# codebydant/sfM_danPipeline

Measured on AMD Instinct MI355X. Metric: image-pairs matched/sec + BA iterations/sec (200 cams, 100k pts, 1M obs), higher is better.
Workload: dtype i8

## Files before the change

### sfm_danpipeline_amd/csrc/match.hip

```cpp
#include "common.h"
#include <type_traits>
#include <vector>
#include <algorithm>
#include <string.h>
#include <stdlib.h>

namespace {

typedef int v4i __attribute__((ext_vector_type(4)));
typedef int v16i __attribute__((ext_vector_type(16)));

enum { KIND_F32_L2 = 0, KIND_U8_L2 = 1, KIND_U8_HAMMING = 2 };

constexpr int TILE_ROWS = 32;
constexpr int HPAD = -(1 << 23);
constexpr int TAG_BITS = 8;
constexpr int EPOCH_TILES = 1 << TAG_BITS;
constexpr int TAG_MASK = EPOCH_TILES - 1;
constexpr int FIX_FLAG = 1 << 30;
constexpr int FIX_GRID = 1024;
constexpr int FIX_CAP = 1 << 20;
constexpr int DIST_EMPTY = 0x7FFFFFFF;
constexpr int KNN_WAVES = 4;
constexpr int HCHUNK = 1024;
// ... 24 lines not shown
  int* par;
  int* nodd;
  int n_rows;
  int n_pad;
};

struct WorkItem {
  int pair;
  int qtile0;
  int qimg, timg;
};

template <int NC>
__host__ __device__ constexpr int chunk_pos(int r, int c) {
  constexpr int SH = (NC == 16) ? 0 : (NC == 8) ? 1 : (NC == 4) ? 2 : 3;
  return r * NC + (c ^ ((r >> SH) & (NC - 1)));
}
__device__ __forceinline__ int imax3(int a, int b, int c) { return max(max(a, b), c); }
__device__ __forceinline__ int imed3(int a, int b, int c) { return max(min(a, b), min(max(a, b), c)); }

template <int KIND>
__global__ __launch_bounds__(256) void parity_kernel(const ImgDev* __restrict__ imgs, const int* __restrict__ tile_img,
                                                     const int* __restrict__ tile_first, int dim) {
  const int img = tile_img[blockIdx.x];
  const int tile = blockIdx.x - tile_first[img];
  const ImgDev I = imgs[img];
  const int l = threadIdx.x & 31;
#pragma unroll
  for (int rr = 0; rr < 4; ++rr) {
    const int row = tile * TILE_ROWS + rr * 8 + (threadIdx.x >> 5);
    int s = 0;
    if (row < I.n_rows) {
      if (KIND == KIND_F32_L2) {
        const float* src = (const float*)I.raw + (size_t)row * dim;
        for (int k = l; k < dim; k += 32) {
          const float f = src[k];
          int x = (int)f;
          x = x < 0 ? 0 : (x > 255 ? 255 : x);
          s ^= x;
        }
      } else {
        const unsigned char* src = (const unsigned char*)I.raw + (size_t)row * dim;
        for (int k = l; k < dim; k += 32) s ^= src[k];
      }
    }
#pragma unroll
    for (int o = 1; o < 32; o <<= 1) s ^= __shfl_xor(s, o);
    if (l == 0 && row < I.n_pad) I.par[row] = (row < I.n_rows) ? (s & 1) : 0;
  }
}

__global__ __launch_bounds__(256) void order_kernel(const ImgDev* __restrict__ imgs, int by_parity) {
  __shared__ int wsum[4];
  __shared__ int run_odd, run_even, n_odd_pad_s;
  const ImgDev I = imgs[blockIdx.x];
  const int lane = threadIdx.x & 63, wave = threadIdx.x >> 6;
  for (int p = threadIdx.x; p < I.n_pad; p += 256) I.perm[p] = (!by_parity && p < I.n_rows) ? p : -1;
  if (!by_parity) {
    if (threadIdx.x == 0) *I.nodd = 0;
    return;
  }
  int c = 0;
  for (int r = threadIdx.x; r < I.n_rows; r += 256) c += I.par[r];
#pragma unroll
  for (int o = 1; o < 64; o <<= 1) c += __shfl_xor(c, o);
  if (lane == 0) wsum[wave] = c;
  __syncthreads();
  if (threadIdx.x == 0) {
    const int n_odd = wsum[0] + wsum[1] + wsum[2] + wsum[3];
    n_odd_pad_s = (n_odd + TILE_ROWS - 1) / TILE_ROWS * TILE_ROWS;
    *I.nodd = n_odd_pad_s;
    run_odd = 0;
    run_even = 0;
  }
  __syncthreads();
  const int n_odd_pad = n_odd_pad_s;
  for (int r0 = 0; r0 < I.n_rows; r0 += 256) {
    const int r = r0 + threadIdx.x;
    const bool valid = r < I.n_rows;
    const bool odd = valid && I.par[r];
    const unsigned long long bo = __ballot(odd), bv = __ballot(valid);
    const unsigned long long below = (1ull << lane) - 1ull;
    if (lane == 0) wsum[wave] = __popcll(bo) | (__popcll(bv) << 16);
    __syncthreads();
    int odd_before = run_odd, valid_before = 0;
    for (int w = 0; w < wave; ++w) {
      odd_before += wsum[w] & 0xFFFF;
      valid_before += wsum[w] >> 16;
    }
    const int my_odd = odd_before + __popcll(bo & below);
    const int my_valid = valid_before + __popcll(bv & below);
    if (valid) {
      const int even_before = run_even + (my_valid - (my_odd - run_odd));
      I.perm[odd ? my_odd : n_odd_pad + even_before] = r;
    }
    __syncthreads();
    if (threadIdx.x == 0) {
      int so = 0, sv = 0;
      for (int w = 0; w < 4; ++w) {
        so += wsum[w] & 0xFFFF;
        sv += wsum[w] >> 16;
      }
      run_odd += so;
      run_even += sv - so;
    }
    __syncthreads();
  }
}

template <int KS, int KIND>
__global__ void prepare_kernel(const ImgDev* __restrict__ imgs, const int* __restrict__ tile_img,
                               const int* __restrict__ tile_first, int dim, int* __restrict__ nonintegral,
                               int gen) {
  constexpr int NC = 2 * KS;
  constexpr int RB = 32 * KS;
  const int img = tile_img[blockIdx.x];
  const int tile = blockIdx.x - tile_first[img];
  const ImgDev I = imgs[img];
  const int r = threadIdx.x / NC, c = threadIdx.x % NC;
  const int pos = tile * TILE_ROWS + r;
  const int row = I.perm[pos];
  const bool valid = row >= 0;
  signed char v[16];
  int n2 = 0;
  bool ok = true;
  if (KIND == KIND_U8_HAMMING) {
    const int nbits = dim * 8;
    unsigned bits = 0;
    if (valid) {
      const unsigned char* src = (const unsigned char*)I.raw + (size_t)row * dim;
      const int b0 = 2 * c;
      if (b0 < dim) bits |= src[b0];
      if (b0 + 1 < dim) bits |= (unsigned)src[b0 + 1] << 8;
    }
#pragma unroll
    for (int e = 0; e < 16; ++e) {
      const int k = c * 16 + e;
      v[e] = (valid && k < nbits) ? (((bits >> e) & 1u) ? 8 : -8) : 0;
    }
  } else {
    float fv[16];
    unsigned char bv[16];
    const bool full = valid && c * 16 + 16 <= dim;
    if (KIND == KIND_F32_L2) {
      const float* src = (const float*)I.raw + (size_t)(valid ? row : 0) * dim + c * 16;
      if (full && (((size_t)src) & 15) == 0) {
        typedef float v4f __attribute__((ext_vector_type(4)));
// ... 15 lines not shown
      if (full && (((size_t)src) & 15) == 0) {
        const v4i x = *(g_v4i_p)src;
        memcpy(bv, &x, 16);
      } else {
#pragma unroll
        for (int e = 0; e < 16; ++e) bv[e] = (valid && c * 16 + e < dim) ? src[e] : 128;
      }
    }
#pragma unroll
    for (int e = 0; e < 16; ++e) {
      const int k = c * 16 + e;
      int x = 128;
      if (valid && k < dim) {
        if (KIND == KIND_F32_L2) {
          const float f = fv[e];
          ok = ok && (f == rintf(f)) && (f >= 0.f) && (f <= 255.f);
          x = (int)f;
          x = x < 0 ? 0 : (x > 255 ? 255 : x);
        } else {
          x = bv[e];
        }
      }
      const int cv = x - 128;
      v[e] = (signed char)cv;
      n2 += cv * cv;
    }
  }
#pragma unroll
  for (int o = 1; o < NC; o <<= 1) n2 += __shfl_xor(n2, o);
  int4 out;
  memcpy(&out, v, 16);
  int4* dst = (int4*)(I.tiles + (size_t)tile * (TILE_ROWS * RB)) + chunk_pos<NC>(r, c);
  *dst = out;
  if (c == 0) {
    int ci;
    if (KIND == KIND_U8_HAMMING)
      ci = ((valid ? dim * 8 * (HCHUNK / 2) : (dim * 8 + 1) * HCHUNK)) | (pos & (HCHUNK - 1));
    else ci = valid ? -((n2 + 1) >> 1) : HPAD;
    I.cin[pos] = ci;
    I.nq[pos] = valid ? n2 : 0;
  }
  if (KIND == KIND_F32_L2 && !ok) nonintegral[img] = gen;
}

template <int NC>
__device__ __forceinline__ int group_sum(int x) {
  if (NC >= 2) x += __builtin_amdgcn_update_dpp(0, x, 0xB1, 0xF, 0xF, true);
  if (NC >= 4) x += __builtin_amdgcn_update_dpp(0, x, 0x4E, 0xF, 0xF, true);
  if (NC >= 8) x += __builtin_amdgcn_update_dpp(0, x, 0x141, 0xF, 0xF, true);
  if (NC >= 16) x += __builtin_amdgcn_update_dpp(0, x, 0x140, 0xF, 0xF, true);
  return x;
}

struct Best2 {
  int d0, i0, x0, d1, i1, x1;
};
__device__ __forceinline__ bool lex_less(int da, int ia, int db, int ib) { return da < db || (da == db && ia < ib); }
__device__ __forceinline__ void best2_insert(Best2& b, int d, int i, int x) {
  if (lex_less(d, i, b.d0, b.i0)) {
    b.d1 = b.d0;
    b.i1 = b.i0;
    b.x1 = b.x0;
    b.d0 = d;
    b.i0 = i;
    b.x0 = x;
  } else if (lex_less(d, i, b.d1, b.i1)) {
    b.d1 = d;
    b.i1 = i;
    b.x1 = x;
  }
}

template <int I>
__device__ __forceinline__ void epi_op(const v16i& D0, const v16i& D1, int (&sl)[16], int& k0, int& k1, int (&T)[16],
                                       int tag0, int tag1) {
  if constexpr (I < 16) {
    sl[I] = imax3(sl[I], D0[I], D1[I]);
  } else {
    constexpr int J = (I - 16) % 11;
    constexpr int B = (I - 16) < 11 ? 0 : 8;
    const v16i& D = (I - 16) < 11 ? D0 : D1;
    const int tag = (I - 16) < 11 ? tag0 : tag1;
    if constexpr (J == 0) T[B + 0] = imax3(D[0], D[1], D[2]);
    if constexpr (J == 1) T[B + 1] = imax3(D[3], D[4], D[5]);
    if constexpr (J == 2) T[B + 2] = imax3(D[6], D[7], D[8]);
    if constexpr (J == 3) T[B + 3] = imax3(D[9], D[10], D[11]);
    if constexpr (J == 4) T[B + 4] = imax3(D[12], D[13], D[14]);
    if constexpr (J == 5) T[B + 5] = imax3(T[B + 0], T[B + 1], T[B + 2]);
    if constexpr (J == 6) T[B + 6] = imax3(T[B + 3], T[B + 4], D[15]);
    if constexpr (J == 7) T[B + 7] = max(T[B + 5], T[B + 6]);
    if constexpr (J == 8) T[B + 7] = (T[B + 7] << TAG_BITS) | tag;
    if constexpr (J == 9) k1 = imed3(k0, k1, T[B + 7]);
    if constexpr (J == 10) k0 = max(k0, T[B + 7]);
  }
}
constexpr int EPI_ORDER[38] = {16, 17, 18, 19, 20, 21, 22, 23, 24, 25, 26, 27, 28, 29, 30, 31, 0, 1,  2,
                                          32, 33, 3,  4,  5,  34, 6,  7,  8,  9,  35, 10, 11, 12, 13, 36, 37, 14, 15};
template <int LO, int HI>
__device__ __forceinline__ void epi_range(const v16i& D0, const v16i& D1, int (&sl)[16], int& k0, int& k1, int (&T)[16],
                                          int tag0, int tag1) {
  if constexpr (LO < HI && LO < 38) {
    epi_op<EPI_ORDER[LO]>(D0, D1, sl, k0, k1, T, tag0, tag1);
    epi_range<LO + 1, HI>(D0, D1, sl, k0, k1, T, tag0, tag1);
  }
}

template <int KS, int MODE, int NU, int SR>
__global__ __launch_bounds__(KNN_WAVES * 64, 2) void knn_kernel(const ImgDev* __restrict__ imgs,
                                                         const WorkItem* __restrict__ items,
                                                         const int* __restrict__ nonintegral, int gen, int dim,
                                                         int4* __restrict__ knn, int maxq,
                                                         int* __restrict__ fix_count, int2* __restrict__ fix_items) {
  constexpr int NC = 2 * KS;
  constexpr int RB = 32 * KS;
  constexpr int TILE_BYTES = TILE_ROWS * RB;
  constexpr int STAGE_ROW_BYTES = SR * RB;
  constexpr int NW = KNN_WAVES;
  constexpr int NT = NW * 64;
  constexpr int CIN_COPIES = (SR + NT - 1) / NT;
  constexpr int STAGE_BYTES = STAGE_ROW_BYTES + CIN_COPIES * NT * 4;
  constexpr int TILES = SR / TILE_ROWS;
  constexpr int TP = TILES / 2;
  constexpr int PIECES = STAGE_ROW_BYTES / (NT * 16);
  constexpr int BATCH = KS <= 4 ? 4 : 2;
  constexpr int NG = 2 * KS;
  constexpr int STAGES_PER_EPOCH = EPOCH_TILES / TILES;
  static_assert(PIECES >= 1 && TP >= 2 && TP % 2 == 0 && STAGES_PER_EPOCH % 2 == 0, "stage shape");
  constexpr int SCRATCH_W = 2048 + (TILE_ROWS * RB > 4096 ? TILE_ROWS * RB : 4096);
  constexpr int BUFA_BYTES = STAGE_BYTES > NW * SCRATCH_W ? STAGE_BYTES : NW * SCRATCH_W;
  constexpr int BUFB_BYTES = (NU < 2 || STAGE_BYTES > NW * SCRATCH_W) ? STAGE_BYTES : NW * SCRATCH_W;
  __shared__ __attribute__((aligned(16))) unsigned char ldsA[BUFA_BYTES];
  __shared__ __attribute__((aligned(16))) unsigned char ldsB[BUFB_BYTES];

  const WorkItem it = items[blockIdx.x];
  if ((nonintegral[it.qimg] == gen) | (nonintegral[it.timg] == gen)) return;
  const ImgDev Q = imgs[it.qimg];
  const ImgDev T = imgs[it.timg];
  const int lane = threadIdx.x & 63;
  const int wave = __builtin_amdgcn_readfirstlane(threadIdx.x >> 6);
  const int r = lane & 31, h = lane >> 5;
  const int nqt = Q.n_pad / TILE_ROWS;
  int qt[NU], qtc[NU];
#pragma unroll
  for (int u = 0; u < NU; ++u) {
    qt[u] = it.qtile0 + NU * wave + u;
    qtc[u] = qt[u] < Q.n_pad / TILE_ROWS ? qt[u] : (Q.n_pad >= TILE_ROWS ? Q.n_pad / TILE_ROWS - 1 : 0);
  }
  SFM_STAMP(0);
  int dbg_trips = 0;

  v4i bq[NU][KS];
#pragma unroll
  for (int u = 0; u < NU; ++u) {
    g_v4i_p src = (g_v4i_p)(Q.tiles + (size_t)qtc[u] * TILE_BYTES);
#pragma unroll
    for (int ks = 0; ks < KS; ++ks) bq[u][ks] = src[chunk_pos<NC>(r, 2 * ks + h)];
  }

  int aoff[KS];
#pragma unroll
  for (int ks = 0; ks < KS; ++ks) aoff[ks] = chunk_pos<NC>(r, 2 * ks + h) * 16;
  const int coff = STAGE_ROW_BYTES + h * 16;

  const int nstages = T.n_pad / SR;
  const int tid = threadIdx.x;

  const __amdgpu_buffer_rsrc_t rs_tiles = __builtin_amdgcn_make_buffer_rsrc((void*)T.tiles, 0, 0x7FFFFFFF, 0x00020000);
  const __amdgpu_buffer_rsrc_t rs_cin = __builtin_amdgcn_make_buffer_rsrc((void*)T.cin, 0, 0x7FFFFFFF, 0x00020000);
  auto stage_copy = [&](int stage, unsigned char* dstb) {
    const int off = stage * STAGE_ROW_BYTES;
#if SFM_DBG == 6
    const unsigned char* src = (const unsigned char*)T.tiles + (size_t)stage * STAGE_ROW_BYTES;
#pragma unroll
    for (int i = 0; i < PIECES; ++i)
      __builtin_amdgcn_global_load_lds((const SFM_GLOBAL void*)(src + (size_t)(i * NT + tid) * 16),
                                       (__attribute__((address_space(3))) void*)(dstb + i * (NT * 16) + wave * 1024), 16, 0, 0);
#pragma unroll
    for (int i = 0; i < CIN_COPIES; ++i)
      __builtin_amdgcn_global_load_lds((const SFM_GLOBAL void*)(T.cin + (size_t)stage * SR + i * NT + tid),
                                       (__attribute__((address_space(3))) void*)(dstb + STAGE_ROW_BYTES + i * (NT * 4) + wave * 256), 4, 0, 0);
    (void)off;
#else
#pragma unroll
    for (int i = 0; i < PIECES; ++i)
      __builtin_amdgcn_raw_ptr_buffer_load_lds(rs_tiles, (__attribute__((address_space(3))) void*)(dstb + i * (NT * 16) + wave * 1024),
                                               16, (i * NT + tid) * 16, off, 0, 0);
#pragma unroll
    for (int i = 0; i < CIN_COPIES; ++i)
      __builtin_amdgcn_raw_ptr_buffer_load_lds(rs_cin, (__attribute__((address_space(3))) void*)(dstb + STAGE_ROW_BYTES + i * (NT * 4) + wave * 256),
                                               4, (i * NT + tid) * 4, stage * SR * 4, 0, 0);
#endif
  };
  auto ld_afrag = [&](const unsigned char* tb, int ks) -> v4i {
    const int4 x = *(const int4*)(tb + aoff[ks]);
    return v4i{x.x, x.y, x.z, x.w};
  };
  auto ld_cin = [&](const unsigned char* sb, int tl, v16i& C) {
#pragma unroll
    for (int g = 0; g < 4; ++g) {
      const int4 x = *(const int4*)(sb + coff + (tl * TILE_ROWS + 8 * g) * 4);
      C[4 * g] = x.x;
      C[4 * g + 1] = x.y;
      C[4 * g + 2] = x.z;
      C[4 * g + 3] = x.w;
    }
  };

  const int nodd_t = MODE == 0 ? *(g_i32_p)T.nodd : 0;
  const int nbits = dim * 8;

  for (int ep0 = 0; ep0 < nstages; ep0 += STAGES_PER_EPOCH) {
    const int ep1 = (ep0 + STAGES_PER_EPOCH < nstages) ? ep0 + STAGES_PER_EPOCH : nstages;
    const int ep_tile0 = ep0 * TILES;
    int sl[NU][16], k0[NU], k1[NU];
#pragma unroll
    for (int u = 0; u < NU; ++u) {
      k0[u] = k1[u] = (int)0x80000000;
#pragma unroll
      for (int e = 0; e < 16; ++e) sl[u][e] = HPAD;
    }
    if (ep0 > 0) __syncthreads();
    stage_copy(ep0, ldsA);
    asm volatile("s_waitcnt vmcnt(0)" ::: "memory");
    __syncthreads();

    v4i F0[KS], F1[KS];
    v16i C0, C1, X0, X1, Y0, Y1;
    int TT[16];
    {
      const unsigned char* sb = ldsA;
#pragma unroll
      for (int ks = 0; ks < KS; ++ks) F0[ks] = ld_afrag(sb, ks);
      ld_cin(sb, 0, C0);
#pragma unroll
      for (int e = 0; e < 16; ++e) X0[e] = X1[e] = Y0[e] = Y1[e] = HPAD;
    }
    int tag = EPOCH_TILES - 1 + 2;
    SFM_STAMP(1);

#define SFM_CHAIN(FA, FB, UF, DA, DB, UD, LD1, SB1, T1, LD0, SB0, T0)                                       \
  do {                                                                                                      \
    _Pragma("unroll") for (int g_ = 0; g_ < NG; ++g_) {                                                     \
      const int ks_ = g_ % KS;                                                                              \
// ... 1 lines not shown
        if (g_ < KS) FA[ks_] += F0[ks_][0] + C0[ks_];                                                       \
        else FB[ks_] += F1[ks_][0] + C1[ks_];                                                               \
      } else if (g_ < KS) FA = __builtin_amdgcn_mfma_i32_32x32x32_i8(F0[ks_], bq[UF][ks_], ks_ == 0 ? C0 : FA, 0, 0, 0); \
      else FB = __builtin_amdgcn_mfma_i32_32x32x32_i8(F1[ks_], bq[UF][ks_], ks_ == 0 ? C1 : FB, 0, 0, 0);  \
      if ((LD1) && g_ == 0) {                                                                               \
        _Pragma("unroll") for (int k2_ = 0; k2_ < KS; ++k2_) F1[k2_] = ld_afrag((SB1) + (T1) * TILE_BYTES, k2_); \
        ld_cin(SB1, T1, C1);                                                                                \
      }                                                                                                     \
      if ((LD0) && g_ < KS) {                                                                               \
        F0[ks_] = ld_afrag((SB0) + (T0) * TILE_BYTES, ks_);                                                 \
        if (g_ == 0) ld_cin(SB0, T0, C0);                                                                   \
      }                                                                                                     \
      if (SFM_DBG != 2) switch (g_) {                                                                       \
        SFM_EPI_CASES(DA, DB, UD)                                                                           \
      }                                                                                                     \
      __builtin_amdgcn_sched_barrier(0);                                                                    \
    }                                                                                                       \
  } while (0)
#define SFM_EPI_CASE(G, DA, DB, UD) \
  case G: epi_range<(G) * 38 / NG, ((G) + 1) * 38 / NG>(DA, DB, sl[UD], k0[UD], k1[UD], TT, tag & TAG_MASK, (tag - 1) & TAG_MASK); break;
#define SFM_EPI_CASES(DA, DB, UD)                                                                          \
  SFM_EPI_CASE(0, DA, DB, UD) SFM_EPI_CASE(1, DA, DB, UD) SFM_EPI_CASE(2, DA, DB, UD) SFM_EPI_CASE(3, DA, DB, UD)     \
  SFM_EPI_CASE(4, DA, DB, UD) SFM_EPI_CASE(5, DA, DB, UD) SFM_EPI_CASE(6, DA, DB, UD) SFM_EPI_CASE(7, DA, DB, UD)     \
  SFM_EPI_CASE(8, DA, DB, UD) SFM_EPI_CASE(9, DA, DB, UD) SFM_EPI_CASE(10, DA, DB, UD) SFM_EPI_CASE(11, DA, DB, UD)   \
  SFM_EPI_CASE(12, DA, DB, UD) SFM_EPI_CASE(13, DA, DB, UD) SFM_EPI_CASE(14, DA, DB, UD) SFM_EPI_CASE(15, DA, DB, UD)

    auto stage = [&](int s, const unsigned char* sb, unsigned char* nb) __attribute__((always_inline)) {
      const bool more = s + 1 < ep1;
      if (more) stage_copy(s + 1, nb);
#pragma unroll
      for (int tp = 0; tp < TP; ++tp) {
        const bool last = tp == TP - 1;
        if (NU == 2) {
          SFM_CHAIN(X0, X1, 0, Y0, Y1, 1, true, sb, 2 * tp + 1, false, sb, 0);
          tag -= 2;
          if (last) {
            asm volatile("s_waitcnt vmcnt(0)" ::: "memory");
            __syncthreads();
          }
          SFM_CHAIN(Y0, Y1, NU - 1, X0, X1, 0, false, sb, 0, true, last ? nb : sb, last ? 0 : 2 * tp + 2);
        } else {
          if (last) {
#pragma unroll
            for (int k2 = 0; k2 < KS; ++k2) F1[k2] = ld_afrag(sb + (2 * tp + 1) * TILE_BYTES, k2);
            ld_cin(sb, 2 * tp + 1, C1);
            asm volatile("s_waitcnt vmcnt(0)" ::: "memory");
            __syncthreads();
          }
          if ((tp & 1) == 0) SFM_CHAIN(X0, X1, 0, Y0, Y1, 0, !last, sb, 2 * tp + 1, true, last ? nb : sb, last ? 0 : 2 * tp + 2);
          else SFM_CHAIN(Y0, Y1, 0, X0, X1, 0, !last, sb, 2 * tp + 1, true, last ? nb : sb, last ? 0 : 2 * tp + 2);
          tag -= 2;
        }
      }
    
    };
    for (int s = ep0; s < ep1; s += 2) {
      stage(s, ldsA, ldsB);
      if (s + 1 < ep1) stage(s + 1, ldsB, ldsA);
    }
    SFM_STAMP(2);
    epi_range<0, 38>(Y0, Y1, sl[NU - 1], k0[NU - 1], k1[NU - 1], TT, tag & TAG_MASK, (tag - 1) & TAG_MASK);
#undef SFM_CHAIN
#undef SFM_EPI_CASES
#undef SFM_EPI_CASE

    int lane_p = lane;
    asm volatile("" : "+v"(lane_p));
    const int r_p = lane_p & 31, h_p = lane_p >> 5;
    typedef __attribute__((address_space(3))) int* lds_vi_p;
#define SFM_WAVE_LDS_FENCE() do { __builtin_amdgcn_fence(__ATOMIC_RELEASE, "wavefront"); __builtin_amdgcn_wave_barrier(); __builtin_amdgcn_fence(__ATOMIC_ACQUIRE, "wavefront"); } while (0)
    __attribute__((address_space(3))) unsigned char* wq[NU];
#pragma unroll
    for (int u = 0; u < NU; ++u)
      wq[u] = (__attribute__((address_space(3))) unsigned char*)(u == 0 ? ldsA : ldsB) + wave * SCRATCH_W + 2048;
    const lds_vi_p wl = (lds_vi_p)(wq[0] - 2048);
    const lds_vi_p wr = NU == 1 ? wl + 256 : (lds_vi_p)(wq[NU - 1] - 2048);
#pragma unroll
    for (int u = 0; u < NU; ++u)
#pragma unroll
      for (int ks = 0; ks < KS; ++ks)
        *(__attribute__((address_space(3))) v4i*)(wq[u] + chunk_pos<NC>(r_p, 2 * ks + h_p) * 16) = bq[u][ks];
    constexpr int SH = (NC == 16) ? 0 : (NC == 8) ? 1 : (NC == 4) ? 2 : 3;
    int cpos[NU][4], chv[NU][4], slot_[NU][4], count[NU];
    bool cval[NU][4], cload[NU][4];
    int qrow[NU], nqq[NU];
    int ovf[NU];
#pragma unroll
    for (int u = 0; u < NU; ++u) {
      const int q = qtc[u] * TILE_ROWS + r_p;
      qrow[u] = ((g_i32_p)Q.perm)[q];
      nqq[u] = ((g_i32_p)Q.nq)[q];
      if (qt[u] >= nqt) qrow[u] = -1;
    }
#pragma unroll
    for (int u = 0; u < NU; ++u) {
      const int bv0 = k0[u] >> TAG_BITS, bv1 = k1[u] >> TAG_BITS;
      const int tl0 = ep_tile0 + (EPOCH_TILES - 1) - (k0[u] & TAG_MASK);
      const int tl1 = ep_tile0 + (EPOCH_TILES - 1) - (k1[u] & TAG_MASK);
      const int pb0 = __shfl_xor(bv0, 32), pb1 = __shfl_xor(bv1, 32);
      int a0 = (HPAD - 1) * 16, a1 = a0, a2 = a0;
#pragma unroll
      for (int e = 0; e < 16; ++e) {
        const int key = (int)((unsigned)sl[u][e] << 4) | e;
        a2 = imed3(a1, a2, key);
        a1 = imed3(a0, a1, key);
        a0 = max(a0, key);
      }
      const int S0 = a0 >> 4, S1 = a1 >> 4, S2 = a2 >> 4;
      const int e0 = a0 & 15, e1 = a1 & 15;
      const int thr = max(max(min(bv0, pb0), max(bv1, pb1)), S1);
      const int ns = (S0 >= thr ? 1 : 0) + (S1 >= thr ? 1 : 0) + (S2 >= thr ? 1 : 0);
      const bool t0in = bv0 >= thr && bv0 > HPAD, t1in = bv1 >= thr && bv1 > HPAD;
      const int rho0 = 8 * (e0 >> 2) + 4 * h_p + (e0 & 3), rho1 = ns >= 2 ? 8 * (e1 >> 2) + 4 * h_p + (e1 & 3) : rho0;
      int over = (ns > 2 && (t0in || t1in)) ? 1 : 0;
      over |= __shfl_xor(over, 32);
      ovf[u] = over;
      const bool known = ns == 1;
      cpos[u][0] = tl0 * TILE_ROWS + rho0;
      cpos[u][1] = tl0 * TILE_ROWS + rho1;
      cpos[u][2] = tl1 * TILE_ROWS + rho0;
      cpos[u][3] = tl1 * TILE_ROWS + rho1;
      cval[u][0] = t0in && ns >= 1;
      cval[u][1] = t0in && ns >= 2;
      cval[u][2] = t1in && ns >= 1;
      cval[u][3] = t1in && ns >= 2;
      chv[u][0] = known ? bv0 : HPAD - 1;
      chv[u][1] = HPAD - 1;
      chv[u][2] = known ? bv1 : HPAD - 1;
      chv[u][3] = HPAD - 1;
      bool need[4] = {!known, !known, !known, !known};
#if SFM_RESOLVE_V2
      if (ns == 2 && S0 != S1 && t0in) {
        const bool gt = S1 > bv1, eq = S1 == bv1, lt = S1 < bv1;
        const bool e1_in = gt || (eq && tl0 < tl1);
        const bool first0 = rho0 < rho1;
        cval[u][0] = true, chv[u][0] = bv0, need[0] = false;
        cval[u][1] = e1_in, chv[u][1] = S1, need[1] = e1_in && !gt;
        cval[u][2] = eq || lt, chv[u][2] = bv1, need[2] = eq && first0;
        cval[u][3] = eq, chv[u][3] = bv1, need[3] = eq && !first0;
      }
#endif
#pragma unroll
      for (int k = 0; k < 4; ++k) {
        cval[u][k] = cval[u][k] && cpos[u][k] < T.n_pad;
        cload[u][k] = cval[u][k] && need[k] && SFM_DBG != 1;
      }
    }
    SFM_STAMP(8);
    int total = 0;
#pragma unroll
    for (int u = 0; u < NU; ++u) {
#pragma unroll
      for (int k = 0; k < 4; ++k) {
        const unsigned long long bm = __ballot(cload[u][k]);
        slot_[u][k] = total + __popcll(bm & ((1ull << lane_p) - 1ull));
        if (cload[u][k]) wl[slot_[u][k]] = cpos[u][k] | (r_p << 26) | (u << 31);
        total += __popcll(bm);
      }
      count[u] = total;
    }
    SFM_WAVE_LDS_FENCE();
    SFM_STAMP(9);
#if SFM_DBG == 4
    if (blockIdx.x < 4096 && lane == 0) {
      g_stamps[(blockIdx.x * 8 + wave) * 16 + 13] = count[0];
      g_stamps[(blockIdx.x * 8 + wave) * 16 + 7] = total - count[0];
    }
#endif
// ... 18 lines not shown
          const __attribute__((address_space(3))) unsigned char* qrw = ((NU > 1 && (ent >> 31)) ? wq[NU - 1] : wq[0]) + qr * (unsigned)RB;
#pragma unroll
          for (int i = 0; i < CPL; ++i) {
            const unsigned p_ = (unsigned)(c + i * LPR);
            xt[st][i] = *(g_v4i_p)(trow + p_ * 16);
            xq[st][i] = *(const __attribute__((address_space(3))) v4i*)(qrw + ((p_ ^ x) << 4));
          }
          ci[st] = ((g_i32_p)T.cin)[ps];
        }
        SFM_STAMP(11);
#if SFM_DBG == 4
        asm volatile("s_waitcnt vmcnt(0)" ::: "memory");
        SFM_STAMP(12);
#endif
#pragma unroll
        for (int st = 0; st < NS; ++st) {
          int dot = 0;
#pragma unroll
          for (int i = 0; i < CPL; ++i)
#pragma unroll
            for (int w = 0; w < 4; ++w) dot = __builtin_amdgcn_sdot4(xt[st][i][w], xq[st][i][w], dot, false);
          dot = group_sum<LPR>(dot) + ci[st];
          wr[(j0 + st * RPS + grp) & (NU * 256 - 1)] = dot;
        }
      };
      for (int j0 = 0; j0 < total; j0 += RPS * STEPS) {
        ++dbg_trips;
        const int left = total - j0;
        if (STEPS >= 4 && left <= RPS * (STEPS / 4)) trip(j0, std::integral_constant<int, (STEPS >= 4 ? STEPS / 4 : 1)>{});
        else if (STEPS >= 2 && left <= RPS * (STEPS / 2)) trip(j0, std::integral_constant<int, (STEPS >= 2 ? STEPS / 2 : 1)>{});
        else if (STEPS >= 4 && left <= RPS * (3 * STEPS / 4)) trip(j0, std::integral_constant<int, (STEPS >= 4 ? 3 * STEPS / 4 : 1)>{});
        else trip(j0, std::integral_constant<int, STEPS>{});
      }
    }
    SFM_WAVE_LDS_FENCE();
    SFM_STAMP(10);
    long long lane_dk[NU][2];
#pragma unroll
    for (int u = 0; u < NU; ++u) {
      long long key[4];
#pragma unroll
      for (int k = 0; k < 4; ++k) {
        if (cload[u][k]) chv[u][k] = wr[slot_[u][k]];
        const int hv = cval[u][k] ? chv[u][k] : HPAD - 1;
        key[k] = ((long long)hv << 32) | (unsigned)(0x7FFFFFFF - cpos[u][k]);
      }
      const long long a = max(key[0], key[1]), b = min(key[0], key[1]);
      const long long c = max(key[2], key[3]), dd = min(key[2], key[3]);
      const long long lk[2] = {max(a, c), max(min(a, c), max(b, dd))};
#pragma unroll
      for (int k = 0; k < 2; ++k) {
        const int hv = (int)(lk[k] >> 32), ps = 0x7FFFFFFF - (int)(unsigned)lk[k];
        const int d = MODE == 0 ? nqq[u] - 2 * hv - (ps < nodd_t ? 1 : 0) : (nbits - hv) >> 1;
        lane_dk[u][k] = hv > HPAD ? (((long long)d << 32) | (unsigned)ps) : 0x7FFFFFFFFFFFFFFFll;
      }
    }
    constexpr bool SPLIT = NU == 2;
    const bool um = SPLIT && h_p != 0;
    long long mine[2], give[2];
#pragma unroll
    for (int k = 0; k < 2; ++k) {
      mine[k] = um ? lane_dk[NU - 1][k] : lane_dk[0][k];
      give[k] = SPLIT ? (um ? lane_dk[0][k] : lane_dk[NU - 1][k]) : lane_dk[0][k];
    }
    const long long o0 = __shfl_xor(give[0], 32), o1 = __shfl_xor(give[1], 32);
    const long long best0 = min(mine[0], o0), best1 = min(max(mine[0], o0), min(mine[1], o1));
    const int my_qrow = um ? qrow[NU - 1] : qrow[0];
    int my_ovf = um ? ovf[NU - 1] : ovf[0];
    const unsigned p0 = (unsigned)best0, p1 = (unsigned)best1;
    const int px0 = ((g_i32_p)T.perm)[p0 < (unsigned)T.n_pad ? p0 : 0u];
    const int px1 = ((g_i32_p)T.perm)[p1 < (unsigned)T.n_pad ? p1 : 0u];
    {
      Best2 m;
      m.d0 = (int)(best0 >> 32), m.i0 = (int)(unsigned)best0, m.x0 = px0;
      m.d1 = (int)(best1 >> 32), m.i1 = (int)(unsigned)best1, m.x1 = px1;
      if (best0 == 0x7FFFFFFFFFFFFFFFll || m.x0 < 0) m.d0 = DIST_EMPTY, m.i0 = 0x7FFFFFFF, m.x0 = -1;
      if (best1 == 0x7FFFFFFFFFFFFFFFll || m.x1 < 0) m.d1 = DIST_EMPTY, m.i1 = 0x7FFFFFFF, m.x1 = -1;
      if ((SPLIT || h_p == 0) && my_qrow >= 0) {
        int4* dst = &knn[(size_t)it.pair * maxq + my_qrow];
        if (ep0 > 0) {
          const int4 pv = *dst;
          Best2 a;
          a.d0 = pv.z, a.x0 = pv.x, a.i0 = -2, a.d1 = pv.w, a.x1 = pv.y, a.i1 = -1;
          if (pv.y == FIX_FLAG) my_ovf = 1;
          if (m.d0 != DIST_EMPTY) best2_insert(a, m.d0, m.i0, m.x0);
          if (m.d1 != DIST_EMPTY) best2_insert(a, m.d1, m.i1, m.x1);
          m = a;
        }
        int4 o;
        if (ep1 < nstages) {
          o.x = m.x0;
          o.y = my_ovf ? FIX_FLAG : m.x1;
          o.z = m.d0;
          o.w = m.d1;
        } else {
          const bool v0 = m.d0 != DIST_EMPTY, v1 = m.d1 != DIST_EMPTY;
          float d0, d1;
          int fix = 0;
          if (MODE == 0) {
            d0 = sqrtf((float)m.d0);
            d1 = sqrtf((float)m.d1);
            if (v1 && m.d1 >= (1 << 22)) fix = FIX_FLAG;
          } else {
            d0 = (float)m.d0;
            d1 = (float)m.d1;
          }
          o.x = v0 ? m.x0 : -1;
          o.y = v1 ? (m.x1 | fix) : -1;
          if (my_ovf) o.y = FIX_FLAG;
          o.z = __float_as_int(v0 ? d0 : 3.402823466e+38f);
          o.w = __float_as_int(v1 ? d1 : 3.402823466e+38f);
          if (o.y >= 0 && (o.y & FIX_FLAG)) {
            const int k = atomicAdd(fix_count, 1);
            if (k < FIX_CAP) fix_items[k] = make_int2(it.pair, my_qrow);
          }
        }
        *dst = o;
      }
    }
    SFM_STAMP(3);
    SFM_STAMP(4);
  }

  SFM_STAMP(5);
#if SFM_DBG == 4
  if (blockIdx.x < 4096 && lane == 0) {
    g_stamps[(blockIdx.x * 8 + wave) * 16 + 14] = __builtin_amdgcn_s_getreg((4 << 0) | (0 << 6) | (31 << 11));
    g_stamps[(blockIdx.x * 8 + wave) * 16 + 15] = __builtin_amdgcn_s_getreg((20 << 0) | (0 << 6) | (31 << 11));
  }
  if (blockIdx.x < 4096 && lane == 0) g_stamps[(blockIdx.x * 8 + wave) * 16 + 6] = dbg_trips;
// ... 740 lines not shown
  hipEvent_t ev_k = nullptr;
  bool timed = false;
  bool pipe_on = false;
  hipStream_t pipe_st = nullptr;
  hipEvent_t ev_ready = nullptr, ev_host[2] = {nullptr, nullptr};
  void* h_pipe[2] = {nullptr, nullptr};
  int* d_pipe[2] = {nullptr, nullptr};
  long long pipe_copied[2] = {0, 0};
  long long pipe_est = -1;
  long long pipe_capacity = 0;
  long long runs = 0;
};

static int pick_ks(int kind, int dim) {
  if (kind == KIND_U8_HAMMING) {
    const int bits = dim * 8;
    if (bits <= 256) return 8;
    return 0;
  }
  if (dim <= 32) return 1;
  if (dim <= 64) return 2;
  if (dim <= 128) return 4;
  if (dim <= 256) return 8;
  return 0;
}

extern "C" int sfmhip_imageset_create(sfmhip_ctx* ctx, int n_images, const int32_t* n_rows, int dim,
                                      int dtype, int norm, sfmhip_imageset** out) {
  if (!ctx || !out || n_images <= 0 || !n_rows || dim <= 0) return SFMHIP_ERR_ARG;
  if (dtype != SFMHIP_F32 && dtype != SFMHIP_U8) return SFMHIP_ERR_ARG;
  if (norm != SFMHIP_L2 && norm != SFMHIP_HAMMING) return SFMHIP_ERR_ARG;
  if (norm == SFMHIP_HAMMING && dtype != SFMHIP_U8) return SFMHIP_ERR_ARG;
  SFM_HIP_TRY(hipSetDevice(ctx->device));
  sfmhip_imageset* s = new sfmhip_imageset();
  s->ctx = ctx;
  s->n_images = n_images;
  s->dim = dim;
  s->dtype = dtype;
  s->norm = norm;
  s->kind = norm == SFMHIP_HAMMING ? KIND_U8_HAMMING : (dtype == SFMHIP_F32 ? KIND_F32_L2 : KIND_U8_L2);
  s->ks = pick_ks(s->kind, dim);
  s->sr = s->ks == 8 ? 128 : 256;
  s->nu = s->ks == 8 ? 1 : 2;
  if (s->kind == KIND_U8_HAMMING) s->nu = 2;
  const int rb = 32 * (s->ks ? s->ks : 1);
  size_t tot_pad = 0;
  std::vector<int> tile_img, tile_first(n_images + 1, 0);
  for (int i = 0; i < n_images; ++i) {
    if (n_rows[i] < 0) {
      delete s;
      return SFMHIP_ERR_ARG;
    }
    s->n_rows.push_back(n_rows[i]);
    const int need = n_rows[i] ? n_rows[i] + (s->kind == KIND_U8_HAMMING ? 0 : TILE_ROWS - 1) : 0;
    const int pad = (need + s->sr - 1) / s->sr * s->sr;
    if ((size_t)pad * rb >= (1ull << 31)) {
      delete s;
      return SFMHIP_ERR_ARG;
    }
    s->n_pad.push_back(pad);
    s->maxq = std::max(s->maxq, n_rows[i]);
    tile_first[i] = (int)tile_img.size();
    for (int t = 0; t < pad / TILE_ROWS; ++t) tile_img.push_back(i);
    tot_pad += pad;
  }
  tile_first[n_images] = (int)tile_img.size();
  s->total_tiles = (int)tile_img.size();
  int rc = SFMHIP_OK;
  if ((rc = sfm_dev_alloc(&s->d_imgs, (size_t)n_images)) || (rc = sfm_dev_alloc(&s->d_tiles, tot_pad * rb)) ||
      (rc = sfm_dev_alloc(&s->d_cin, tot_pad + 512)) || (rc = sfm_dev_alloc(&s->d_nq, tot_pad)) ||
      (rc = sfm_dev_alloc(&s->d_perm, tot_pad)) || (rc = sfm_dev_alloc(&s->d_par, tot_pad)) ||
      (rc = sfm_dev_alloc(&s->d_nodd, (size_t)n_images)) ||
      (rc = sfm_dev_alloc(&s->d_tile_img, tile_img.size())) ||
      (rc = sfm_dev_alloc(&s->d_tile_first, (size_t)n_images + 1)) ||
      (rc = sfm_dev_alloc(&s->d_nonintegral, (size_t)n_images))) {
    sfmhip_imageset_destroy(s);
    return rc;
  }
#define SFM_HIP_TRY_OR_DESTROY(expr, obj, destroy)                                        \
  do {                                                                                    \
    hipError_t e__ = (expr);                                                              \
    if (e__ != hipSuccess) {                                                              \
      g_sfmhip_last_hip_error = (int)e__;                                                 \
      fprintf(stderr, "[sfmhip] %s:%d %s -> %s\n", __FILE__, __LINE__, #expr, hipGetErrorString(e__)); \
      destroy(obj);                                                                       \
      return SFMHIP_ERR_HIP;                                                              \
    }                                                                                     \
  } while (0)
  SFM_HIP_TRY_OR_DESTROY(hipMemcpy(s->d_tile_img, tile_img.data(), tile_img.size() * sizeof(int), hipMemcpyHostToDevice), s,
                         sfmhip_imageset_destroy);
  SFM_HIP_TRY_OR_DESTROY(hipMemcpy(s->d_tile_first, tile_first.data(), tile_first.size() * sizeof(int), hipMemcpyHostToDevice), s,
                         sfmhip_imageset_destroy);
  SFM_HIP_TRY_OR_DESTROY(hipMemset(s->d_nonintegral, 0xFF, n_images * sizeof(int)), s, sfmhip_imageset_destroy);
  s->h_imgs.resize(n_images);
  s->owned_raw.assign(n_images, nullptr);
  size_t off = 0;
  for (int i = 0; i < n_images; ++i) {
    ImgDev& I = s->h_imgs[i];
    I.raw = nullptr;
    I.tiles = s->d_tiles + off * rb;
    I.cin = s->d_cin + off;
    I.nq = s->d_nq + off;
    I.perm = s->d_perm + off;
    I.par = s->d_par + off;
    I.nodd = s->d_nodd + i;
    I.n_rows = s->n_rows[i];
    I.n_pad = s->n_pad[i];
    off += s->n_pad[i];
// ... 57 lines not shown
  }
  const bool timing = s->ctx->timing;
  if (timing) SFM_HIP_TRY(hipEventRecord(s->ev_prep0, st));
  ++s->gen;
  if (s->total_tiles > 0) {
    switch (s->ks) {
      case 1: launch_prepare<1>(s); break;
      case 2: launch_prepare<2>(s); break;
      case 4: launch_prepare<4>(s); break;
      case 8: launch_prepare<8>(s); break;
      default: break;
    }
    SFM_HIP_TRY(hipGetLastError());
  }
  if (timing) SFM_HIP_TRY(hipEventRecord(s->ev_prep1, st));
  s->prep_timed = timing;
  return SFMHIP_OK;
}

extern "C" void sfmhip_imageset_destroy(sfmhip_imageset* s) {
  if (!s) return;
  hipSetDevice(s->ctx->device);
  for (void* p : s->owned_raw)
    if (p) hipFree(p);
  hipFree(s->d_imgs);
  hipFree(s->d_tiles);
  hipFree(s->d_cin);
  hipFree(s->d_nq);
  hipFree(s->d_perm);
  hipFree(s->d_par);
  hipFree(s->d_nodd);
  hipFree(s->d_tile_img);
  hipFree(s->d_tile_first);
  hipFree(s->d_nonintegral);
  if (s->ev_prep0) hipEventDestroy(s->ev_prep0);
  if (s->ev_prep1) hipEventDestroy(s->ev_prep1);
  delete s;
}

static void build_work_items(const sfmhip_imageset* s, const int32_t* pairs, int n_pairs, std::vector<WorkItem>& items) {
  std::vector<WorkItem> lanes[8];
  std::vector<int> order(n_pairs);
  for (int p = 0; p < n_pairs; ++p) order[p] = p;
  std::stable_sort(order.begin(), order.end(), [&](int a, int b) { return pairs[2 * a + 1] < pairs[2 * b + 1]; });
  size_t load[8] = {0, 0, 0, 0, 0, 0, 0, 0};
  int cur_t = -1, cur_lane = 0;
  for (int p : order) {
    const int qi = pairs[2 * p], ti = pairs[2 * p + 1];
    if (s->n_rows[ti] < 1 || s->n_rows[qi] == 0) continue;
    if (ti != cur_t) {
      cur_t = ti;
      cur_lane = (int)(std::min_element(load, load + 8) - load);
    }
    const int npos = s->n_rows[qi] + (s->kind == KIND_U8_HAMMING ? 0 : TILE_ROWS - 1);
    const int nqt = std::min((npos + TILE_ROWS - 1) / TILE_ROWS, s->n_pad[qi] / TILE_ROWS);
    for (int t0 = 0; t0 < nqt; t0 += KNN_WAVES * s->nu) {
      lanes[cur_lane].push_back(WorkItem{p, t0, qi, ti});
      load[cur_lane] += (size_t)s->n_pad[ti];
    }
  }
  items.clear();
  size_t mx = 0;
  for (auto& l : lanes) mx = std::max(mx, l.size());
  std::vector<size_t> pos(8, 0);
  for (size_t i = 0; i < mx; ++i)
    for (int x = 0; x < 8; ++x)
      if (pos[x] < lanes[x].size()) items.push_back(lanes[x][pos[x]++]);
}

static int plan_check_pairs(const sfmhip_imageset* s, const int32_t* pairs, int n_pairs) {
  for (int p = 0; p < n_pairs; ++p)
    if (pairs[2 * p] < 0 || pairs[2 * p] >= s->n_images || pairs[2 * p + 1] < 0 || pairs[2 * p + 1] >= s->n_images)
      return SFMHIP_ERR_ARG;
  return SFMHIP_OK;
}

extern "C" int sfmhip_matchplan_create(sfmhip_imageset* s, const int32_t* pairs, int n_pairs, sfmhip_matchplan** out) {
  if (!s || !out || n_pairs < 0 || (n_pairs && !pairs)) return SFMHIP_ERR_ARG;
  SFM_HIP_TRY(hipSetDevice(s->ctx->device));
  SFM_TRY(plan_check_pairs(s, pairs, n_pairs));
  sfmhip_matchplan* pl = new sfmhip_matchplan();
  pl->set = s;
  pl->n_pairs = n_pairs;
  pl->cap_pairs = std::max(n_pairs, 1);
  pl->maxq = std::max(s->maxq, 1);
  pl->h_pairs.assign(pairs, pairs + 2 * (size_t)n_pairs);
  std::vector<WorkItem> items;
  build_work_items(s, pairs, n_pairs, items);
  pl->n_items = (int)items.size();
  pl->cap_items = (size_t)pl->cap_pairs * (size_t)(((pl->maxq + 2 * TILE_ROWS - 2) / TILE_ROWS + KNN_WAVES * s->nu - 1) / (KNN_WAVES * s->nu));
  int rc = SFMHIP_OK;
  const size_t slots = (size_t)pl->cap_pairs * pl->maxq;
  if ((rc = sfm_dev_alloc(&pl->d_pairs, (size_t)pl->cap_pairs)) || (rc = sfm_dev_alloc(&pl->d_items, pl->cap_items)) ||
      (rc = sfm_dev_alloc(&pl->d_knn, slots)) || (rc = sfm_dev_alloc(&pl->d_counts, (size_t)pl->cap_pairs)) ||
      (rc = sfm_dev_alloc(&pl->d_out_q, slots)) || (rc = sfm_dev_alloc(&pl->d_out_t, slots)) ||
      (rc = sfm_dev_alloc(&pl->d_out_d, slots)) || (rc = sfm_dev_alloc(&pl->d_fix_count, (size_t)1)) ||
      (rc = sfm_dev_alloc(&pl->d_fix_items, (size_t)FIX_CAP)) || (rc = sfm_dev_alloc(&pl->d_fix_part, (size_t)FIX_GRID)) ||
      (rc = sfm_dev_alloc(&pl->d_fix_arrived, (size_t)FIX_GRID))) {
    sfmhip_matchplan_destroy(pl);
    return rc;
  }
  if (n_pairs) SFM_HIP_TRY_OR_DESTROY(hipMemcpy(pl->d_pairs, pairs, sizeof(int2) * n_pairs, hipMemcpyHostToDevice), pl, sfmhip_matchplan_destroy);
  if (!items.empty())
    SFM_HIP_TRY_OR_DESTROY(hipMemcpy(pl->d_items, items.data(), sizeof(WorkItem) * items.size(), hipMemcpyHostToDevice), pl,
                           sfmhip_matchplan_destroy);
  SFM_HIP_TRY_OR_DESTROY(hipMemset(pl->d_counts, 0, sizeof(int) * pl->cap_pairs), pl, sfmhip_matchplan_destroy);
  SFM_HIP_TRY_OR_DESTROY(hipMemset(pl->d_fix_count, 0, sizeof(int)), pl, sfmhip_matchplan_destroy);
  SFM_HIP_TRY_OR_DESTROY(hipMemset(pl->d_fix_arrived, 0, sizeof(int) * FIX_GRID), pl, sfmhip_matchplan_destroy);
  for (auto& e : pl->ev) SFM_HIP_TRY_OR_DESTROY(hipEventCreate(&e), pl, sfmhip_matchplan_destroy);
  SFM_HIP_TRY_OR_DESTROY(hipEventCreate(&pl->ev_k), pl, sfmhip_matchplan_destroy);
  *out = pl;
  return SFMHIP_OK;
}

extern "C" int sfmhip_matchplan_set_pairs(sfmhip_matchplan* pl, const int32_t* pairs, int n_pairs) {
  if (!pl || n_pairs < 0 || (n_pairs && !pairs) || n_pairs > pl->cap_pairs) return SFMHIP_ERR_ARG;
  sfmhip_imageset* s = pl->set;
  SFM_HIP_TRY(hipSetDevice(s->ctx->device));
  SFM_TRY(plan_check_pairs(s, pairs, n_pairs));
  std::vector<WorkItem> items;
  build_work_items(s, pairs, n_pairs, items);
  if (items.size() > pl->cap_items) return SFMHIP_ERR_STATE;
  hipStream_t st = s->ctx->stream;
  SFM_HIP_TRY(hipStreamSynchronize(st));
  if (pl->pipe_st) SFM_HIP_TRY(hipStreamSynchronize(pl->pipe_st));
  pl->n_pairs = n_pairs;
  pl->n_items = (int)items.size();
  pl->h_pairs.assign(pairs, pairs + 2 * (size_t)n_pairs);
  if (n_pairs) SFM_HIP_TRY(hipMemcpyAsync(pl->d_pairs, pairs, sizeof(int2) * n_pairs, hipMemcpyHostToDevice, st));
  if (!items.empty())
    SFM_HIP_TRY(hipMemcpyAsync(pl->d_items, items.data(), sizeof(WorkItem) * items.size(), hipMemcpyHostToDevice, st));
  SFM_HIP_TRY(hipMemsetAsync(pl->d_counts, 0, sizeof(int) * pl->cap_pairs, st));
  SFM_HIP_TRY(hipStreamSynchronize(st));
  pl->timed = false;
  return SFMHIP_OK;
}

template <int KS, int MODE, int NU, int SR>
static int launch_knn(sfmhip_matchplan* pl) {
  sfmhip_imageset* s = pl->set;
  hipLaunchKernelGGL((knn_kernel<KS, MODE, NU, SR>), dim3(pl->n_items), dim3(KNN_WAVES * 64), 0, s->ctx->stream, s->d_imgs,
                     pl->d_items, s->d_nonintegral, s->gen, s->dim, pl->d_knn, pl->maxq, pl->d_fix_count, pl->d_fix_items);
  SFM_HIP_TRY(hipGetLastError());
// ... 337 lines not shown
```

Measured before the change: 2.058 million.

## Drop parity/tile padding and add partial-stage tail path in kNN kernel

Removes the extra padding rows that split odd and even parity groups, and sizes image padding and query tile counts from real row counts. The kNN kernel now runs full stages only up to the last complete stage and handles the leftover tiles with a new tail routine, instead of processing padded stages. This is meant to skip MFMA work on padding rows. Cross-half shuffles become ds_bpermute and buffer-load offsets are hoisted into scalar operands. It adds a complex macro-based tail path with reversed epilogue ordering, which carries correctness risk.

```diff
diff --git a/sfm_danpipeline_amd/csrc/match.hip b/sfm_danpipeline_amd/csrc/match.hip
--- a/sfm_danpipeline_amd/csrc/match.hip
+++ b/sfm_danpipeline_amd/csrc/match.hip
@@ -100,7 +100,7 @@
 
 __global__ __launch_bounds__(256) void order_kernel(const ImgDev* __restrict__ imgs, int by_parity) {
   __shared__ int wsum[4];
-  __shared__ int run_odd, run_even, n_odd_pad_s;
+  __shared__ int run_odd, run_even, n_odd_s;
   const ImgDev I = imgs[blockIdx.x];
   const int lane = threadIdx.x & 63, wave = threadIdx.x >> 6;
   for (int p = threadIdx.x; p < I.n_pad; p += 256) I.perm[p] = (!by_parity && p < I.n_rows) ? p : -1;
@@ -116,13 +116,13 @@
   __syncthreads();
   if (threadIdx.x == 0) {
     const int n_odd = wsum[0] + wsum[1] + wsum[2] + wsum[3];
-    n_odd_pad_s = (n_odd + TILE_ROWS - 1) / TILE_ROWS * TILE_ROWS;
-    *I.nodd = n_odd_pad_s;
+    n_odd_s = n_odd;
+    *I.nodd = n_odd;
     run_odd = 0;
     run_even = 0;
   }
   __syncthreads();
-  const int n_odd_pad = n_odd_pad_s;
+  const int n_odd = n_odd_s;
   for (int r0 = 0; r0 < I.n_rows; r0 += 256) {
     const int r = r0 + threadIdx.x;
     const bool valid = r < I.n_rows;
@@ -140,7 +140,7 @@
     const int my_valid = valid_before + __popcll(bv & below);
     if (valid) {
       const int even_before = run_even + (my_valid - (my_odd - run_odd));
-      I.perm[odd ? my_odd : n_odd_pad + even_before] = r;
+      I.perm[odd ? my_odd : n_odd + even_before] = r;
     }
     __syncthreads();
     if (threadIdx.x == 0) {
@@ -262,6 +262,11 @@
   return x;
 }
 
+__device__ __forceinline__ int lane_id_here() {
+  int l;
+  asm volatile("v_mbcnt_lo_u32_b32 %0, -1, 0\n\tv_mbcnt_hi_u32_b32 %0, -1, %0" : "=v"(l));
+  return l;
+}
 struct Best2 {
   int d0, i0, x0, d1, i1, x1;
 };
@@ -306,12 +311,13 @@
 }
 constexpr int EPI_ORDER[38] = {16, 17, 18, 19, 20, 21, 22, 23, 24, 25, 26, 27, 28, 29, 30, 31, 0, 1,  2,
                                           32, 33, 3,  4,  5,  34, 6,  7,  8,  9,  35, 10, 11, 12, 13, 36, 37, 14, 15};
-template <int LO, int HI>
+constexpr int epi_swap_trees(int id) { return id < 16 ? id : (id < 27 ? id + 11 : id - 11); }
+template <int LO, int HI, bool REV = false>
 __device__ __forceinline__ void epi_range(const v16i& D0, const v16i& D1, int (&sl)[16], int& k0, int& k1, int (&T)[16],
                                           int tag0, int tag1) {
   if constexpr (LO < HI && LO < 38) {
-    epi_op<EPI_ORDER[LO]>(D0, D1, sl, k0, k1, T, tag0, tag1);
-    epi_range<LO + 1, HI>(D0, D1, sl, k0, k1, T, tag0, tag1);
+    epi_op<REV ? epi_swap_trees(EPI_ORDER[LO]) : EPI_ORDER[LO]>(D0, D1, sl, k0, k1, T, tag0, tag1);
+    epi_range<LO + 1, HI, REV>(D0, D1, sl, k0, k1, T, tag0, tag1);
   }
 }
 
@@ -349,12 +355,12 @@
   const int lane = threadIdx.x & 63;
   const int wave = __builtin_amdgcn_readfirstlane(threadIdx.x >> 6);
   const int r = lane & 31, h = lane >> 5;
-  const int nqt = Q.n_pad / TILE_ROWS;
+  const int nqt = (Q.n_rows + TILE_ROWS - 1) / TILE_ROWS;
   int qt[NU], qtc[NU];
 #pragma unroll
   for (int u = 0; u < NU; ++u) {
     qt[u] = it.qtile0 + NU * wave + u;
-    qtc[u] = qt[u] < Q.n_pad / TILE_ROWS ? qt[u] : (Q.n_pad >= TILE_ROWS ? Q.n_pad / TILE_ROWS - 1 : 0);
+    qtc[u] = qt[u] < nqt ? qt[u] : (nqt > 0 ? nqt - 1 : 0);
   }
   SFM_STAMP(0);
   int dbg_trips = 0;
@@ -372,7 +378,9 @@
   for (int ks = 0; ks < KS; ++ks) aoff[ks] = chunk_pos<NC>(r, 2 * ks + h) * 16;
   const int coff = STAGE_ROW_BYTES + h * 16;
 
-  const int nstages = T.n_pad / SR;
+  const int tiles_t = (T.n_rows + TILE_ROWS - 1) / TILE_ROWS;
+  const int nfull = tiles_t / TILES, tail_tiles = tiles_t % TILES;
+  const int nstages = nfull + (tail_tiles ? 1 : 0);
   const int tid = threadIdx.x;
 
   const __amdgpu_buffer_rsrc_t rs_tiles = __builtin_amdgcn_make_buffer_rsrc((void*)T.tiles, 0, 0x7FFFFFFF, 0x00020000);
@@ -391,14 +399,15 @@
                                        (__attribute__((address_space(3))) void*)(dstb + STAGE_ROW_BYTES + i * (NT * 4) + wave * 256), 4, 0, 0);
     (void)off;
 #else
+    const int tid16 = (wave * 64 + lane_id_here()) * 16;
 #pragma unroll
     for (int i = 0; i < PIECES; ++i)
       __builtin_amdgcn_raw_ptr_buffer_load_lds(rs_tiles, (__attribute__((address_space(3))) void*)(dstb + i * (NT * 16) + wave * 1024),
-                                               16, (i * NT + tid) * 16, off, 0, 0);
+                                               16, tid16, off + i * (NT * 16), 0, 0);
 #pragma unroll
     for (int i = 0; i < CIN_COPIES; ++i)
       __builtin_amdgcn_raw_ptr_buffer_load_lds(rs_cin, (__attribute__((address_space(3))) void*)(dstb + STAGE_ROW_BYTES + i * (NT * 4) + wave * 256),
-                                               4, (i * NT + tid) * 4, stage * SR * 4, 0, 0);
+                                               4, (int)((unsigned)tid16 >> 2), (stage * SR + i * NT) * 4, 0, 0);
 #endif
   };
   auto ld_afrag = [&](const unsigned char* tb, int ks) -> v4i {
@@ -506,21 +515,89 @@
           tag -= 2;
         }
       }
-    
+
     };
-    for (int s = ep0; s < ep1; s += 2) {
+#define SFM_TAIL_CHAIN(B1, B2, UF, DA, DB, UD, DREV, SB, T2, LDC, TC, LDF, TF, HALF)                        \
+  do {                                                                                                      \
+    if (HALF) {                                                                                             \
+      int hp_ = HPAD;                                                                                       \
+      asm volatile("" : "+v"(hp_));  \
+      _Pragma("unroll") for (int e_ = 0; e_ < 16; ++e_) B2[e_] = hp_;                                       \
+    } else ld_cin(SB, T2, B2);                                                                              \
+    _Pragma("unroll") for (int g_ = 0; g_ < NG; ++g_) {                                                     \
+      const int ks_ = g_ % KS;                                                                              \
+      if (SFM_DBG == 3) {                                                                                   \
+      } else if (g_ < KS) B1 = __builtin_amdgcn_mfma_i32_32x32x32_i8(F0[ks_], bq[UF][ks_], ks_ == 0 ? C0 : B1, 0, 0, 0); \
+      else if (!(HALF)) B2 = __builtin_amdgcn_mfma_i32_32x32x32_i8(F0[ks_], bq[UF][ks_], B2, 0, 0, 0);      \
+      if (!(HALF) && g_ < KS) F0[ks_] = ld_afrag((SB) + (T2) * TILE_BYTES, ks_);                            \
+      if ((LDC) && g_ == 0) ld_cin(SB, TC, C0);                                                             \
+      if ((LDF) && g_ >= KS) F0[ks_] = ld_afrag((SB) + (TF) * TILE_BYTES, ks_);                             \
+      if (SFM_DBG != 2) switch (g_) {                                                                       \
+        SFM_EPI_CASES_R(DA, DB, UD, DREV)                                                                   \
+      }                                                                                                     \
+      __builtin_amdgcn_sched_barrier(0);                                                                    \
+    }                                                                                                       \
+  } while (0)
+#define SFM_EPI_CASE_R(G, DA, DB, UD, DREV) \
+  case G: epi_range<(G) * 38 / NG, ((G) + 1) * 38 / NG, DREV>(DA, DB, sl[UD], k0[UD], k1[UD], TT, tag & TAG_MASK, (tag - 1) & TAG_MASK); break;
+#define SFM_EPI_CASES_R(DA, DB, UD, R)                                                                       \
+  SFM_EPI_CASE_R(0, DA, DB, UD, R) SFM_EPI_CASE_R(1, DA, DB, UD, R) SFM_EPI_CASE_R(2, DA, DB, UD, R) SFM_EPI_CASE_R(3, DA, DB, UD, R)     \
+  SFM_EPI_CASE_R(4, DA, DB, UD, R) SFM_EPI_CASE_R(5, DA, DB, UD, R) SFM_EPI_CASE_R(6, DA, DB, UD, R) SFM_EPI_CASE_R(7, DA, DB, UD, R)     \
+  SFM_EPI_CASE_R(8, DA, DB, UD, R) SFM_EPI_CASE_R(9, DA, DB, UD, R) SFM_EPI_CASE_R(10, DA, DB, UD, R) SFM_EPI_CASE_R(11, DA, DB, UD, R)   \
+  SFM_EPI_CASE_R(12, DA, DB, UD, R) SFM_EPI_CASE_R(13, DA, DB, UD, R) SFM_EPI_CASE_R(14, DA, DB, UD, R) SFM_EPI_CASE_R(15, DA, DB, UD, R)
+    auto tail = [&](const unsigned char* sb) __attribute__((always_inline)) {
+      const int npairs = tail_tiles >> 1;
+#pragma nounroll
+      for (int tp = 0; tp < npairs; ++tp) {
+        if (NU == 2) {
+          SFM_TAIL_CHAIN(X0, X1, 0, Y0, Y1, 1, true, sb, 2 * tp + 1, true, 2 * tp + 1, false, 0, false);
+          tag -= 2;
+          SFM_TAIL_CHAIN(Y1, Y0, NU - 1, X0, X1, 0, false, sb, 2 * tp, true, 2 * tp + 2, true, 2 * tp + 2, false);
+        } else {
+          SFM_TAIL_CHAIN(X0, X1, 0, Y0, Y1, 0, false, sb, 2 * tp + 1, true, 2 * tp + 2, true, 2 * tp + 2, false);
+          tag -= 2;
+          Y0 = X0;
+          Y1 = X1;
+        }
+      }
+      if (tail_tiles & 1) {
+        SFM_TAIL_CHAIN(X0, X1, 0, Y0, Y1, NU - 1, NU == 2, sb, 0, false, 0, false, 0, true);
+        tag -= 2;
+        if (NU == 2) {
+          SFM_TAIL_CHAIN(Y0, Y1, NU - 1, X0, X1, 0, false, sb, 0, false, 0, false, 0, true);
+        } else {
+          Y0 = X0;
+          Y1 = X1;
+        }
+      }
+      __syncthreads();
+    };
+    const int epf = ep1 < nfull ? ep1 : nfull;
+    for (int s = ep0; s < epf; s += 2) {
       stage(s, ldsA, ldsB);
-      if (s + 1 < ep1) stage(s + 1, ldsB, ldsA);
-    }
+      if (s + 1 < epf) stage(s + 1, ldsB, ldsA);
+    }
+    if (epf < ep1) tail((nfull & 1) == 0 ? (const unsigned char*)ldsA : (const unsigned char*)ldsB);
     SFM_STAMP(2);
     epi_range<0, 38>(Y0, Y1, sl[NU - 1], k0[NU - 1], k1[NU - 1], TT, tag & TAG_MASK, (tag - 1) & TAG_MASK);
 #undef SFM_CHAIN
+#undef SFM_TAIL_CHAIN
+#undef SFM_EPI_CASES_R
+#undef SFM_EPI_CASE_R
 #undef SFM_EPI_CASES
 #undef SFM_EPI_CASE
 
-    int lane_p = lane;
-    asm volatile("" : "+v"(lane_p));
+    const int lane_p = lane_id_here();
     const int r_p = lane_p & 31, h_p = lane_p >> 5;
+    const int partner4 = (lane_p ^ 32) << 2;
+    auto xor32 = [&](int x) -> int { return __builtin_amdgcn_ds_bpermute(partner4, x); };
+    auto xor32ll = [&](long long x) -> long long {
+      const unsigned lo = (unsigned)xor32((int)(unsigned)x), hi = (unsigned)xor32((int)(x >> 32));
+      return (long long)(((unsigned long long)hi << 32) | lo);
+    };
+    int none_lo, none_hi;
+    asm volatile("v_mov_b32 %0, -1\n\tv_bfrev_b32 %1, -2" : "=v"(none_lo), "=v"(none_hi));
+    const long long dk_none = (long long)(((unsigned long long)(unsigned)none_hi << 32) | (unsigned)none_lo);
     typedef __attribute__((address_space(3))) int* lds_vi_p;
 #define SFM_WAVE_LDS_FENCE() do { __builtin_amdgcn_fence(__ATOMIC_RELEASE, "wavefront"); __builtin_amdgcn_wave_barrier(); __builtin_amdgcn_fence(__ATOMIC_ACQUIRE, "wavefront"); } while (0)
     __attribute__((address_space(3))) unsigned char* wq[NU];
@@ -551,7 +628,7 @@
       const int bv0 = k0[u] >> TAG_BITS, bv1 = k1[u] >> TAG_BITS;
       const int tl0 = ep_tile0 + (EPOCH_TILES - 1) - (k0[u] & TAG_MASK);
       const int tl1 = ep_tile0 + (EPOCH_TILES - 1) - (k1[u] & TAG_MASK);
-      const int pb0 = __shfl_xor(bv0, 32), pb1 = __shfl_xor(bv1, 32);
+      const int pb0 = xor32(bv0), pb1 = xor32(bv1);
       int a0 = (HPAD - 1) * 16, a1 = a0, a2 = a0;
 #pragma unroll
       for (int e = 0; e < 16; ++e) {
@@ -567,7 +644,7 @@
       const bool t0in = bv0 >= thr && bv0 > HPAD, t1in = bv1 >= thr && bv1 > HPAD;
       const int rho0 = 8 * (e0 >> 2) + 4 * h_p + (e0 & 3), rho1 = ns >= 2 ? 8 * (e1 >> 2) + 4 * h_p + (e1 & 3) : rho0;
       int over = (ns > 2 && (t0in || t1in)) ? 1 : 0;
-      over |= __shfl_xor(over, 32);
+      over |= xor32(over);
       ovf[u] = over;
       const bool known = ns == 1;
       cpos[u][0] = tl0 * TILE_ROWS + rho0;
@@ -692,7 +769,7 @@
       for (int k = 0; k < 2; ++k) {
         const int hv = (int)(lk[k] >> 32), ps = 0x7FFFFFFF - (int)(unsigned)lk[k];
         const int d = MODE == 0 ? nqq[u] - 2 * hv - (ps < nodd_t ? 1 : 0) : (nbits - hv) >> 1;
-        lane_dk[u][k] = hv > HPAD ? (((long long)d << 32) | (unsigned)ps) : 0x7FFFFFFFFFFFFFFFll;
+        lane_dk[u][k] = hv > HPAD ? (((long long)d << 32) | (unsigned)ps) : dk_none;
       }
     }
     constexpr bool SPLIT = NU == 2;
@@ -703,7 +780,7 @@
       mine[k] = um ? lane_dk[NU - 1][k] : lane_dk[0][k];
       give[k] = SPLIT ? (um ? lane_dk[0][k] : lane_dk[NU - 1][k]) : lane_dk[0][k];
     }
-    const long long o0 = __shfl_xor(give[0], 32), o1 = __shfl_xor(give[1], 32);
+    const long long o0 = xor32ll(give[0]), o1 = xor32ll(give[1]);
     const long long best0 = min(mine[0], o0), best1 = min(max(mine[0], o0), min(mine[1], o1));
     const int my_qrow = um ? qrow[NU - 1] : qrow[0];
     int my_ovf = um ? ovf[NU - 1] : ovf[0];
@@ -714,8 +791,8 @@
       Best2 m;
       m.d0 = (int)(best0 >> 32), m.i0 = (int)(unsigned)best0, m.x0 = px0;
       m.d1 = (int)(best1 >> 32), m.i1 = (int)(unsigned)best1, m.x1 = px1;
-      if (best0 == 0x7FFFFFFFFFFFFFFFll || m.x0 < 0) m.d0 = DIST_EMPTY, m.i0 = 0x7FFFFFFF, m.x0 = -1;
-      if (best1 == 0x7FFFFFFFFFFFFFFFll || m.x1 < 0) m.d1 = DIST_EMPTY, m.i1 = 0x7FFFFFFF, m.x1 = -1;
+      if (best0 == dk_none || m.x0 < 0) m.d0 = DIST_EMPTY, m.i0 = 0x7FFFFFFF, m.x0 = -1;
+      if (best1 == dk_none || m.x1 < 0) m.d1 = DIST_EMPTY, m.i1 = 0x7FFFFFFF, m.x1 = -1;
       if ((SPLIT || h_p == 0) && my_qrow >= 0) {
         int4* dst = &knn[(size_t)it.pair * maxq + my_qrow];
         if (ep0 > 0) {
@@ -1562,8 +1639,7 @@
       return SFMHIP_ERR_ARG;
     }
     s->n_rows.push_back(n_rows[i]);
-    const int need = n_rows[i] ? n_rows[i] + (s->kind == KIND_U8_HAMMING ? 0 : TILE_ROWS - 1) : 0;
-    const int pad = (need + s->sr - 1) / s->sr * s->sr;
+    const int pad = (n_rows[i] + s->sr - 1) / s->sr * s->sr;
     if ((size_t)pad * rb >= (1ull << 31)) {
       delete s;
       return SFMHIP_ERR_ARG;
@@ -1727,8 +1803,7 @@
       cur_t = ti;
       cur_lane = (int)(std::min_element(load, load + 8) - load);
     }
-    const int npos = s->n_rows[qi] + (s->kind == KIND_U8_HAMMING ? 0 : TILE_ROWS - 1);
-    const int nqt = std::min((npos + TILE_ROWS - 1) / TILE_ROWS, s->n_pad[qi] / TILE_ROWS);
+    const int nqt = (s->n_rows[qi] + TILE_ROWS - 1) / TILE_ROWS;
     for (int t0 = 0; t0 < nqt; t0 += KNN_WAVES * s->nu) {
       lanes[cur_lane].push_back(WorkItem{p, t0, qi, ti});
       load[cur_lane] += (size_t)s->n_pad[ti];
@@ -1763,7 +1838,7 @@
   std::vector<WorkItem> items;
   build_work_items(s, pairs, n_pairs, items);
   pl->n_items = (int)items.size();
-  pl->cap_items = (size_t)pl->cap_pairs * (size_t)(((pl->maxq + 2 * TILE_ROWS - 2) / TILE_ROWS + KNN_WAVES * s->nu - 1) / (KNN_WAVES * s->nu));
+  pl->cap_items = (size_t)pl->cap_pairs * (size_t)(((pl->maxq + TILE_ROWS - 1) / TILE_ROWS + KNN_WAVES * s->nu - 1) / (KNN_WAVES * s->nu));
   int rc = SFMHIP_OK;
   const size_t slots = (size_t)pl->cap_pairs * pl->maxq;
   if ((rc = sfm_dev_alloc(&pl->d_pairs, (size_t)pl->cap_pairs)) || (rc = sfm_dev_alloc(&pl->d_items, pl->cap_items)) ||
```

Result: no change. 2.050 million (-0.4%).
